# Diamondfan/CTC_pytorch

Measured on AMD Instinct MI355X. Metric: acoustic frames/sec/GPU (train) + utterances/sec beam-decode (`decode` object), TIMIT 4x320 BiLSTM, higher is better.
Workload: dtype f32 via bf16x3 split-operand MFMA (f32 accumulate); 1 GPU; cfg2: 4x320 BiLSTM + BN + Linear(62) + CTC, B=32/GPU, T=800, F=40, dropout 0.1, Adam; global_batch=32, seq_len=800, parallelism=dp1, full_length_utterances=True, sync_bn=False

## Files before the change

### ctc_pytorch_amd/_lib.py

```python
import ctypes
import glob
import os
import subprocess

import torch

_HERE = os.path.dirname(os.path.abspath(__file__))
_CSRC = os.path.join(_HERE, "csrc")
SO_PATH = os.environ.get("CTCN_LIBCTCN") or os.path.join(_HERE, "libctcn.so")
_lib = None

c_void_p, c_int, c_float, c_double, c_size_t, c_u64 = (ctypes.c_void_p, ctypes.c_int, ctypes.c_float,
                                                      ctypes.c_double, ctypes.c_size_t, ctypes.c_uint64)

P, I, F, D, Z, U = c_void_p, c_int, c_float, c_double, c_size_t, c_u64
_SIGS = {
    "ctcn_version": (I, []),
    "ctcn_last_error": (ctypes.c_char_p, []),
    "ctcn_device_cus": (I, []),
    "ctcn_device_xcds": (I, []),
    "ctcn_set_option": (I, [ctypes.c_char_p, I]),
    "ctcn_get_option": (I, [ctypes.c_char_p]),
    "ctcn_option_name": (ctypes.c_char_p, [I]),
    "ctcn_set_status_buffer": (I, [P]),
    "ctcn_gemm": (I, [I, I, I, I, I, P, I, P, I, P, I, F, I, P, Z, P]),
    "ctcn_transpose01": (I, [P, P, I, I, I, P]),
    "ctcn_copy_strided4": (I, [P, P, I, I, I, I, Z, Z, Z, Z, P]),
    "ctcn_relu_fwd": (I, [P, P, Z, P]),
    "ctcn_relu_bwd": (I, [P, P, P, Z, P]),
    "ctcn_maxpool2d_fwd": (I, [P, P, P, Z, I, I, I, I, P]),
    "ctcn_maxpool2d_bwd": (I, [P, P, P, Z, I, I, I, I, P]),
    "ctcn_rnn_scratch_bytes": (Z, [I, I, I, I]),
    "ctcn_rnn_fwd": (I, [I, I, I, I, I, I, P, P, P, P, P, P, P, P, I, P, Z, P]),
    "ctcn_rnn_fwd_dropout": (I, [I, I, I, I, I, I, P, P, P, P, P, P, P, P, P, F, U, U, I, P, Z, P]),
    "ctcn_rnn_bwd": (I, [I, I, I, I, I, I, P, P, P, P, P, P, P, P, P, P, P, P, P, P, F, I, P, P, Z, P]),
    "ctcn_rnn_bwd_dropout": (I, [I, I, I, I, I, I, P, P, P, P, P, P, P, P, P, P, P, P, P, P, F, I, P, P, Z, P, F, U, U, P]),
    "ctcn_rnn_bwd_weights": (I, [I, I, I, I, I, I, P, P, P, P, P, P, P, P, F, I, ctypes.c_uint, P, Z, P]),
    "ctcn_bn_ws_bytes": (Z, [I, I, I]),
    "ctcn_bn_fwd_train": (I, [P, P, P, P, P, P, P, P, I, I, I, F, F, I, P, Z, P, P]),
    "ctcn_bn_fwd_eval": (I, [P, P, P, P, P, P, I, I, I, F, I, P]),
    "ctcn_bn_fwd_sums": (I, [P, P, I, I, I, P, Z, P]),
    "ctcn_bn_fwd_finish": (I, [P, P, P, P, P, P, P, P, P, D, I, I, I, F, F, I, P, P]),
    "ctcn_bn_bwd_sums": (I, [P, P, P, P, P, P, I, I, I, I, P, Z, P]),
    "ctcn_bn_bwd_finish": (I, [P, P, P, P, P, P, P, P, P, P, P, D, I, I, I, I, F, P, Z, P]),
    "ctcn_bn_bwd": (I, [P, P, P, P, P, P, P, P, P, I, I, I, I, F, P, Z, P]),
    "ctcn_bn_fwd_train_dropout": (I, [P, P, P, P, P, P, P, P, I, I, I, F, F, I, P, Z, P, P, F, U, U]),
    "ctcn_bn_bwd_dropout": (I, [P, P, P, P, P, P, P, P, P, I, I, I, I, F, P, Z, P, F, U, U]),
    "ctcn_dropout": (I, [P, P, Z, F, U, U, P]),
    "ctcn_bn_masked_ws_bytes": (Z, [I, I, I]),
    "ctcn_mask_frames": (I, [P, P, P, I, I, I, I, I, P]),
    "ctcn_bn_fwd_train_masked": (I, [P, P, P, P, P, P, P, P, P, I, I, I, I, I, F, F, I, P, Z, P, P]),
    "ctcn_bn_fwd_eval_masked": (I, [P, P, P, P, P, P, P, I, I, I, I, I, F, I, P]),
    "ctcn_bn_bwd_masked": (I, [P, P, P, P, P, P, P, P, P, P, I, I, I, I, I, I, F, P, Z, P]),
    "ctcn_conv2d_ws_bytes": (Z, [I] * 11),
    "ctcn_conv2d_fwd": (I, [P, P, P, P] + [I] * 11 + [P]),
    "ctcn_conv2d_bwd": (I, [P, P, P, P, P, P] + [I] * 11 + [F, P, Z, P]),
    "ctcn_bctf_to_tbcf": (I, [P, P, I, I, I, I, P]),
    "ctcn_tbcf_to_bctf": (I, [P, P, I, I, I, I, P]),
# ... 8 lines not shown
    "ctcn_ctc_grad": (I, [P, P, P, P, P, P, P, P, P, I, I, I, I, P]),
    "ctcn_sum_f32": (I, [P, P, I, P]),
    "ctcn_ctc_fwd_ex": (I, [P, P, P, P, P, P, P, I, I, I, I, I, P]),
    "ctcn_ctc_grad_ex": (I, [P, P, P, P, P, P, P, P, I, I, I, I, P, I, I, I, I, P]),
    "ctcn_ctc_reduce": (I, [P, P, P, I, I, I, P]),
    "ctcn_ctc_pack_targets": (I, [P, ctypes.c_int64, P, P, I, I, P]),
    "ctcn_ctc_align_ws_bytes": (Z, [I, I, I]),
    "ctcn_ctc_align": (I, [P, P, P, P, P, P, P, P, P, P, I, I, I, I, I, P, Z, P]),
    "ctcn_adam_step": (I, [P, P, P, P, Z, F, F, F, F, F, I, P]),
    "ctcn_grad_norm_ws_bytes": (Z, [Z, I]),
    "ctcn_grad_norm": (I, [P, Z, I, P, I, P, P, P, I, P, Z, P]),
    "ctcn_clip_control": (I, [P, F, F, F, F, I, P]),
    "ctcn_adam_step_ex": (I, [P, P, P, P, Z, F, F, F, F, P, P]),
    "ctcn_scale_by_device_scalar": (I, [P, Z, P, P]),
    "ctcn_greedy_collapse": (I, [P, Z, Z, P, P, P, I, I, I, P]),
    "ctcn_path_tokens": (I, [P, Z, Z, P, P, P, P, P, P, P, P, P, P, I, I, I, I, P]),
    "ctcn_edit_distance": (I, [P, P, P, P, P, I, I, I, I, P]),
    "ctcn_edit_ops_ws_bytes": (Z, [I, I, I]),
    "ctcn_edit_ops": (I, [P, P, P, P, P, I, P, P, P, P, I, I, I, I, P, Z, P]),
    "ctcn_step_stats": (I, [P, P, P, I, P, P, P]),
    "ctcn_fbank_frames": (I, [ctypes.c_longlong, I, I, I]),
    "ctcn_fbank_plan_bytes": (Z, [P]),
    "ctcn_fbank_plan": (I, [P, P, Z]),
    "ctcn_fbank": (I, [P, I, P, P, P, P, P, P, P, I, I, I, F, U, U, P]),
    "ctcn_cmvn_accumulate_ws_bytes": (Z, [I, I, I]),
    "ctcn_cmvn_accumulate": (I, [P, P, P, I, I, I, P, Z, P]),
    "ctcn_comm_unique_id": (I, [P]),
    "ctcn_comm_init": (I, [P, I, I, ctypes.POINTER(ctypes.c_void_p)]),
    "ctcn_comm_allreduce_sum_f32": (I, [P, P, Z, P]),
    "ctcn_comm_destroy": (I, [P]),
    "ctcn_diag_squat": (I, [I, I, I, ctypes.c_uint, P]),
    "ctcn_diag_pipeline_chunks": (I, [I, I, I, I, I, I, I, I, ctypes.c_uint]),
    "ctcn_diag_gemm_plan": (I, [I] * 13 + [Z, ctypes.c_uint, I, I, I, I, P]),
    "ctcn_diag_gemm_on_xcds": (I, [I, I, I, I, I, P, I, P, I, P, I, F, I, P, Z, P, ctypes.c_uint]),
    "ctcn_rnn_last_kernel": (ctypes.c_char_p, [I]),
    "ctcn_levenshtein": (ctypes.c_longlong, [P, ctypes.c_longlong, P, ctypes.c_longlong]),
    "ctcn_levenshtein_ops": (ctypes.c_longlong, [P, ctypes.c_longlong, P, ctypes.c_longlong, P, P]),
    "ctcn_join_tokens": (ctypes.c_longlong, [P, ctypes.c_longlong, P, I, P, P, P, I, I, P, ctypes.c_longlong, P]),
    "ctcn_beam_ws_bytes": (Z, [I, I, I, I]),
    "ctcn_beam_decode": (I, [P, I, P, P, D, I, I, P, P, P, P, I, I, I, P, Z, P]),
    "ctcn_beam_decode_nbest": (I, [P, I, P, P, D, I, I, I, P, P, P, P, P, I, I, I, P, Z, P]),
}


class RnnCall(ctypes.Structure):
    _fields_ = [("drop_p", ctypes.c_float), ("drop_seed", ctypes.c_uint64), ("drop_offset", ctypes.c_uint64), ("y_drop", ctypes.c_void_p),
                ("dy_tmp", ctypes.c_void_p), ("side_stream", ctypes.c_void_p), ("side_event", ctypes.c_void_p), ("side_ws", ctypes.c_void_p),
                ("side_ws_bytes", ctypes.c_size_t), ("xcd_allow", ctypes.c_uint), ("prelaunch_event", ctypes.c_void_p), ("status", ctypes.c_void_p),
                ("launched", ctypes.POINTER(ctypes.c_char_p))]


class FbankOpts(ctypes.Structure):
    _fields_ = [(k, ctypes.c_float) for k in ("samp_freq", "frame_shift_ms", "frame_length_ms", "preemph_coeff", "blackman_coeff", "low_freq",
                                              "high_freq", "energy_floor")] + \
               [(k, ctypes.c_int32) for k in ("window_type", "num_mel_bins", "remove_dc_offset", "round_to_power_of_two", "snip_edges",
                                              "use_energy", "raw_energy", "htk_compat", "use_log_fbank", "use_power")]


def sources():
    return sorted(glob.glob(os.path.join(_CSRC, "*.hip")))


def build(force=False, verbose=False):
    from concurrent.futures import ThreadPoolExecutor
    srcs = sources()
    hdrs = glob.glob(os.path.join(_CSRC, "*.h")) + [os.path.join(os.path.dirname(_HERE), "include", "ctcn.h")]
# ... 101 lines not shown
```

### ctc_pytorch_amd/csrc/core.hip

```cpp
#include "common.h"

static thread_local char g_err[512] = "";

void ctcn_set_error(const char *fmt, ...) {
  va_list ap;
  va_start(ap, fmt);
  vsnprintf(g_err, sizeof(g_err), fmt, ap);
  va_end(ap);
}

extern "C" int ctcn_version(void) { return 100; }
extern "C" const char *ctcn_last_error(void) { return g_err; }
extern "C" int ctcn_device_cus(void) {
  int dev = 0, n = 0;
  if (hipGetDevice(&dev) != hipSuccess) return -1;
  if (hipDeviceGetAttribute(&n, hipDeviceAttributeMultiprocessorCount, dev) != hipSuccess) return -1;
  return n;
}

static int g_opt_rnn_persistent = 1;
static int g_opt_handoff = 1;
static int g_opt_poll_depth = 2;
static int g_opt_recurrence_only = 0;
static int g_opt_bwd_scatter = 1;
static int g_opt_handoff_tags = 1;
static int g_opt_side_split_wgs = 8;
static int g_opt_gemm_big_tiles = 0;
static int g_opt_gemm_tile256 = 1;
static int g_opt_gemm_dbg = 0;
static int g_opt_gemm_a_inline = 1;
static int g_opt_conv_mfma = 1;
static int g_opt_rnn_mixed_slices = 0;
static int g_opt_rnn_fwd_tagged = 1;
static int g_opt_rnn_fused_dropout = 1;
static int g_opt_gemm_tn = 1;
static int g_opt_tag_poll_delay = 8;
static int g_opt_edit_wave = 1;
static int g_opt_bwd_item_gather = 1;
static int g_opt_bwd_poll_delay = -1;
static int g_opt_fwd_rsv_lds = 2;
static int g_opt_fwd_pipe_any_chunking = 0;
static int g_opt_fwd_pipe_min_input = 0;
static int g_opt_conv_dbg = 0;
static int g_opt_rnn_rsv_nt = 0;
static int g_opt_gemm_bf16_single = 0;
static int g_opt_xcd_interleave = 1;
static int g_opt_bn_rows4 = 1;
static int g_opt_tn_splits_force = 0;
static int g_opt_tn_splits_xcd = 1;
static int g_opt_beam_generic_threads = 0;
static int g_opt_beam_bitonic = 1;
static int g_opt_beam_cand_global = 0;
static int g_opt_beam_occ2 = 0;
static int g_opt_beam_fast = 1;
static int g_opt_rnn_slow_items = 0;
static int g_opt_rnn_slow_exchange = 0;
static int g_opt_xcd_interleave_force = 0;
static int *g_status_dev = nullptr;

struct OptionRow { const char *name; int *var; int (*norm)(int); };
static const OptionRow k_options[] = {
  {"rnn_persistent", &g_opt_rnn_persistent, [](int value) -> int { return value; }},
  {"handoff", &g_opt_handoff, [](int value) -> int { return value; }},
  {"poll_depth", &g_opt_poll_depth, [](int value) -> int { return value; }},
  {"rnn_recurrence_only", &g_opt_recurrence_only, [](int value) -> int { return value ? 1 : 0; }},
  {"bwd_scatter", &g_opt_bwd_scatter, [](int value) -> int { return value ? 1 : 0; }},
  {"handoff_tags", &g_opt_handoff_tags, [](int value) -> int { return value ? 1 : 0; }},
  {"side_split_wgs", &g_opt_side_split_wgs, [](int value) -> int { return value < 1 ? 1 : (value > 16 ? 16 : value); }},
  {"gemm_big_tiles", &g_opt_gemm_big_tiles, [](int value) -> int { return value ? 1 : 0; }},
  {"beam_fast", &g_opt_beam_fast, [](int value) -> int { return value ? 1 : 0; }},
  {"conv_dbg", &g_opt_conv_dbg, [](int value) -> int { return value & 7; }},
  {"rnn_rsv_nt", &g_opt_rnn_rsv_nt, [](int value) -> int { return value ? 1 : 0; }},
  {"tn_splits_xcd", &g_opt_tn_splits_xcd, [](int value) -> int { return value ? 1 : 0; }},
  {"xcd_interleave", &g_opt_xcd_interleave, [](int value) -> int { return value < 0 ? 0 : (value > 5 ? 5 : value); }},
  {"bn_rows4", &g_opt_bn_rows4, [](int value) -> int { return value ? 1 : 0; }},
  {"tn_splits_force", &g_opt_tn_splits_force, [](int value) -> int { return value < 0 ? 0 : value; }},
  {"gemm_bf16_single", &g_opt_gemm_bf16_single, [](int value) -> int { return value ? 1 : 0; }},
  {"beam_generic_threads", &g_opt_beam_generic_threads, [](int value) -> int { return (value == 256 || value == 512 || value == 1024) ? value : 0; }},
  {"beam_cand_global", &g_opt_beam_cand_global, [](int value) -> int { return value ? 1 : 0; }},
  {"beam_bitonic", &g_opt_beam_bitonic, [](int value) -> int { return value ? 1 : 0; }},
  {"beam_occ2", &g_opt_beam_occ2, [](int value) -> int { return value < 0 ? 0 : (value > 2 ? 2 : value); }},
  {"fwd_pipe_min_input", &g_opt_fwd_pipe_min_input, [](int value) -> int { return value < 0 ? 0 : value; }},
  {"fwd_pipe_any_chunking", &g_opt_fwd_pipe_any_chunking, [](int value) -> int { return value ? 1 : 0; }},
  {"fwd_rsv_lds", &g_opt_fwd_rsv_lds, [](int value) -> int { return value < 0 ? 0 : (value > 2 ? 2 : value); }},
  {"bwd_item_gather", &g_opt_bwd_item_gather, [](int value) -> int { return value < 0 ? 0 : (value > 2 ? 2 : value); }},
  {"bwd_poll_delay", &g_opt_bwd_poll_delay, [](int value) -> int { return value < 0 ? -1 : (value > 256 ? 256 : value); }},
  {"conv_mfma", &g_opt_conv_mfma, [](int value) -> int { return value ? 1 : 0; }},
  {"edit_wave", &g_opt_edit_wave, [](int value) -> int { return value ? 1 : 0; }},
  {"gemm_tn", &g_opt_gemm_tn, [](int value) -> int { return value != 0; }},
  {"rnn_fused_dropout", &g_opt_rnn_fused_dropout, [](int value) -> int { return value != 0; }},
  {"tag_poll_delay", &g_opt_tag_poll_delay, [](int value) -> int { return value < 0 ? 0 : (value > 64 ? 64 : value); }},
  {"rnn_fwd_tagged", &g_opt_rnn_fwd_tagged, [](int value) -> int { return value ? 1 : 0; }},
  {"rnn_mixed_slices", &g_opt_rnn_mixed_slices, [](int value) -> int { return value ? 1 : 0; }},
  {"gemm_a_inline", &g_opt_gemm_a_inline, [](int value) -> int { return value ? 1 : 0; }},
  {"gemm_dbg", &g_opt_gemm_dbg, [](int value) -> int { return value; }},
  {"gemm_tile256", &g_opt_gemm_tile256, [](int value) -> int { return value ? 1 : 0; }},
  {"xcd_interleave_force", &g_opt_xcd_interleave_force, [](int value) -> int { return value ? 1 : 0; }},
  {"rnn_slow_exchange", &g_opt_rnn_slow_exchange, [](int value) -> int { return value < 0 ? 0 : (value > 4096 ? 4096 : value); }},
  {"rnn_slow_items", &g_opt_rnn_slow_items, [](int value) -> int { return value < 0 ? 0 : (value > 4096 ? 4096 : value); }},
};
static const int k_noptions = (int)(sizeof(k_options) / sizeof(k_options[0]));
static const OptionRow *find_option(const char *name) {
  if (name)
    for (int i = 0; i < k_noptions; ++i)
      if (!strcmp(name, k_options[i].name)) return &k_options[i];
  return nullptr;
}
extern "C" int ctcn_set_option(const char *name, int value) {
  if (const OptionRow *o = find_option(name)) { *o->var = o->norm(value); return CTCN_OK; }
  ctcn_set_error("ctcn_set_option: unknown option %s", name ? name : "(null)");
// ... 18 lines not shown
```

### ctc_pytorch_amd/csrc/gemm.hip

```cpp
#include <algorithm>
#include <type_traits>

#include "common.h"

namespace {

constexpr int BM = 128, BN = 128, BK = 16, PAD = 4;

__device__ __forceinline__ int xcd_band_tile(int bid, int nt) {
  const int xcd = bid & 7, q = nt >> 3, r = nt & 7;
  return (xcd < r ? xcd * (q + 1) : r * (q + 1) + (xcd - r) * q) + (bid >> 3);
}
__device__ __forceinline__ void g2r_kc(const float *__restrict__ src, int ld, int r0, int R, int k0, int Kend,
                                       bool vec, int tid, float (&reg)[8]) {
#pragma unroll
  for (int j = 0; j < 2; ++j) {
    const int idx = tid + 256 * j;
    const int r = idx >> 2, kq = (idx & 3) * 4;
    const int gr = r0 + r, gk = k0 + kq;
    const float *p = src + (size_t)gr * ld + gk;
    if (vec && gr < R && gk + 3 < Kend) {
      const float4 v = *reinterpret_cast<const float4 *>(p);
      reg[4 * j + 0] = v.x; reg[4 * j + 1] = v.y; reg[4 * j + 2] = v.z; reg[4 * j + 3] = v.w;
    } else {
// ... 953 lines not shown
    }
#ifdef CTCN_GEMM_STATS
    PPB_VM(2);
#else
    __builtin_amdgcn_sched_barrier(0);
    if constexpr (HAS2) asm volatile("s_waitcnt vmcnt(2) lgkmcnt(0)\n\ts_barrier" ::: "memory");
    else asm volatile("s_waitcnt vmcnt(0) lgkmcnt(0)\n\ts_barrier" ::: "memory");
    __builtin_amdgcn_sched_barrier(0);
#endif
    multiply(second, has1, has2, s);
    PPB(3);
  };
  int s = 0;
  for (; s + 2 < nst; ++s) stage(s, yes, yes);
#ifdef CTCN_GEMM_STATS
  if (lane == 0 && (wave & 3) == 0 && (blockIdx.x == 0 || blockIdx.x == 1000) && g_gemm_stats) {
    long long *o = g_gemm_stats + ((blockIdx.x ? 2 : 0) + (wave >> 2)) * 16;
    for (int i = 0; i < 4; ++i) { o[i] = gs_work[i]; o[4 + i] = gs_wait[i]; }
    o[8] = clock64() - gs_t0; o[9] = nst - 2; o[10] = 0;
  }
#endif
  if (s + 1 < nst) { stage(s, yes, no); ++s; }
  stage(s, no, no);
  if (wm == 0) pp_barrier();
#pragma unroll
  for (int i = 0; i < 4; ++i)
#pragma unroll
    for (int j = 0; j < WNT; ++j) {
      const int col = n0 + wn * 32 * WNT + j * 32 + (lane & 31);
#pragma unroll
      for (int e = 0; e < 16; ++e) {
        const int row = m0 + wm * 128 + i * 32 + (e & 3) + 8 * (e >> 2) + 4 * (lane >> 5);
        if (row < M && col < N) {
          float v = acc[i][j][e];
          float *p = C + (size_t)row * ldc + col;
          if (beta != 0.0f) v += beta * *p;
          *p = v;
        }
      }
    }
}


typedef short s16x4_t __attribute__((ext_vector_type(4)));
typedef short s16x8_t __attribute__((ext_vector_type(8)));

template <int WNT, int NP = 3>
__global__ __launch_bounds__(512) void gemm_tn_f32_pp_kernel(int M, int N, int K, const float *__restrict__ A, int lda, const float *__restrict__ B,
                                                             int ldb, float *__restrict__ C, int ldc, float beta, int kchunk, int splits,
                                                             float *__restrict__ part, int tiles_m, int tiles_n, unsigned xcd_mask,
                                                             unsigned *__restrict__ queue) {
  constexpr int TBM = 256, TBN = 128 * WNT;
  constexpr int A_BYTES = TBM * 64, B_BYTES = TBN * 64;
  constexpr int STAGE = 2 * A_BYTES + 2 * B_BYTES;
  constexpr int NB = 2 * WNT;
  constexpr int NMM = 4 * WNT;
  extern __shared__ __attribute__((aligned(16))) unsigned char qsm[];
  __shared__ int s_item;
  {
    unsigned xcc;
    asm volatile("s_getreg_b32 %0, hwreg(HW_REG_XCC_ID)" : "=s"(xcc));
    if (!((xcd_mask >> (xcc & 15u)) & 1u)) return;
  }
  const int tid = threadIdx.x, lane = tid & 63, wave = __builtin_amdgcn_readfirstlane(tid >> 6);
  const int wm = wave >> 2, wn = wave & 3;
  const int nt = tiles_m * tiles_n;
// ... 560 lines not shown
  return CTCN_OK;
}

int ctcn_gemm_on_xcds(int transA, int transB, int M, int N, int K, const float *A, int lda, const float *B, int ldb, float *C,
                      int ldc, float beta, int precision, void *ws, size_t ws_bytes, void *stream, unsigned xcd_allow, GemmPlanes *planes) {
  return gemm_core(transA, transB, M, N, K, A, lda, B, ldb, C, ldc, beta, precision, ws, ws_bytes, stream, xcd_allow, planes, 0);
}
extern "C" int ctcn_diag_gemm_on_xcds(int transA, int transB, int M, int N, int K, const float *A, int lda, const float *B, int ldb, float *C, int ldc,
                                      float beta, int precision, void *ws, size_t ws_bytes, void *stream, unsigned xcd_allow) {
  return gemm_core(transA, transB, M, N, K, A, lda, B, ldb, C, ldc, beta, precision, ws, ws_bytes, stream, xcd_allow, nullptr, 0);
}

int ctcn_gemm_shift_b(int M, int N, int K, const float *A, int lda, const float *B, int ldb, float *C, int ldc, float beta, int precision,
                      void *ws, size_t ws_bytes, void *stream, unsigned xcd_allow, int shift, GemmPlanes *planes) {
  const int as = shift < 0 ? -shift : shift;
  CTCN_REQUIRE(as < K, "ctcn_gemm_shift_b: |shift| %d >= K %d", as, K);
  const GemmEnv e = {(int)((uintptr_t)A & 15), (int)((uintptr_t)B & 15), ws != nullptr, ws_bytes, xcd_allow, false, false, ctcn_device_cus(), 0, gemm_options()};
  const bool plane = uses_planes(plan_gemm({1, 0, M, N, K, lda, ldb, ldc, precision, shift}, e).path) &&
                     plan_gemm({1, 0, M, N, K - as, lda, ldb, ldc, precision, 0}, e).path != GP_TN;
  if (!plane) {
    if (planes) planes->same_a = false;
    const float *A2 = shift > 0 ? A + (size_t)as * lda : A, *B2 = shift < 0 ? B + (size_t)as * ldb : B;
    return gemm_core(1, 0, M, N, K - as, A2, lda, B2, ldb, C, ldc, beta, precision, ws, ws_bytes, stream, xcd_allow, planes, 0);
  }
  return gemm_core(1, 0, M, N, K, A, lda, B, ldb, C, ldc, beta, precision, ws, ws_bytes, stream, xcd_allow, planes, shift);
}

extern "C" int ctcn_gemm(int transA, int transB, int M, int N, int K, const float *A, int lda, const float *B,
                         int ldb, float *C, int ldc, float beta, int precision, void *ws, size_t ws_bytes,
                         void *stream) {
  return gemm_core(transA, transB, M, N, K, A, lda, B, ldb, C, ldc, beta, precision, ws, ws_bytes, stream, 0u, nullptr, 0);
}

__global__ void transpose01_pair_kernel(const float *__restrict__ in0, const float *__restrict__ in1, float *__restrict__ out0, float *__restrict__ out1,
                                        int A, int B, int C) {
  const float *in = blockIdx.y ? in1 : in0;
  float *out = blockIdx.y ? out1 : out0;
  const size_t total = (size_t)A * B * C;
  for (size_t i = blockIdx.x * (size_t)blockDim.x + threadIdx.x; i < total; i += (size_t)gridDim.x * blockDim.x) {
    const int c = i % C;
    const size_t ab = i / C;
    const int a = ab % A;
    const int b = ab / A;
    out[i] = in[((size_t)a * B + b) * C + c];
  }
}
__global__ __launch_bounds__(256) void transpose2d_pair_kernel(const float *__restrict__ in0, const float *__restrict__ in1, float *__restrict__ out0,
                                                               float *__restrict__ out1, int A, int B) {
  __shared__ float tile[32][33];
  const float *in = blockIdx.z ? in1 : in0;
  float *out = blockIdx.z ? out1 : out0;
  const int tx = threadIdx.x & 31, ty = threadIdx.x >> 5;
  const int b0 = blockIdx.x * 32, a0 = blockIdx.y * 32;
#pragma unroll
  for (int k = 0; k < 4; ++k) {
    const int a = a0 + ty + 8 * k, b = b0 + tx;
    if (a < A && b < B) tile[ty + 8 * k][tx] = in[(size_t)a * B + b];
  }
  __syncthreads();
#pragma unroll
  for (int k = 0; k < 4; ++k) {
    const int b = b0 + ty + 8 * k, a = a0 + tx;
    if (a < A && b < B) out[(size_t)b * A + a] = tile[tx][ty + 8 * k];
  }
}
int ctcn_transpose01_pair(const float *in0, const float *in1, float *out0, float *out1, int A, int B, int C, void *stream) {
// ... 22 lines not shown
```

### ctc_pytorch_amd/csrc/rnn.hip

```cpp
#include <algorithm>
#include <stdlib.h>

#include <atomic>

#include "common.h"
#include <type_traits>

namespace {

__device__ __forceinline__ float act_sigmoid(float x) { return __builtin_amdgcn_rcpf(1.0f + __builtin_amdgcn_exp2f(-1.4426950408889634f * x)); }
__device__ __forceinline__ float act_tanh(float x) {
  const float e = __builtin_amdgcn_exp2f(-2.8853900817779268f * fabsf(x));
  return copysignf((1.0f - e) * __builtin_amdgcn_rcpf(1.0f + e), x);
}

typedef __bf16 bf16x8_t __attribute__((ext_vector_type(8)));
union Bf16Pack { u32x4 u; bf16x8_t v; };
__device__ __forceinline__ void split8(const f32x4 &a, const f32x4 &b, bf16x8_t &hi, bf16x8_t &lo) {
  unsigned h[8], l[8];
#pragma unroll
  for (int e = 0; e < 8; ++e) {
    const float x = e < 4 ? a[e] : b[e - 4];
    h[e] = f2bf(x);
    l[e] = f2bf(x - __uint_as_float(h[e] << 16));
// ... 2371 lines not shown
  bool drop_pending = c.y_drop != nullptr;
  const int rc = rnn_fwd_impl(cell, T, B, I, H, dirs, x, w_ih0, w_hh0, w_ih1, w_hh1, y, gates, aux, precision, ws, ws_bytes, stream, c, drop_pending);
  if (rc) return rc;
  return drop_pending ? ctcn_dropout(y, c.y_drop, (size_t)T * B * dirs * H, c.drop_p, c.drop_seed, c.drop_offset, stream) : CTCN_OK;
}
extern "C" int ctcn_rnn_fwd(int cell, int T, int B, int I, int H, int dirs, const float *x, const float *w_ih0,
                            const float *w_hh0, const float *w_ih1, const float *w_hh1, float *y, float *gates,
                            float *aux, int precision, void *ws, size_t ws_bytes, void *stream) {
  return ctcn_rnn_fwd_ex(cell, T, B, I, H, dirs, x, w_ih0, w_hh0, w_ih1, w_hh1, y, gates, aux, precision, ws, ws_bytes, stream, nullptr);
}
extern "C" int ctcn_rnn_fwd_dropout(int cell, int T, int B, int I, int H, int dirs, const float *x, const float *w_ih0, const float *w_hh0,
                                    const float *w_ih1, const float *w_hh1, float *y, float *gates, float *aux, float *y_drop, float p, uint64_t seed,
                                    uint64_t offset, int precision, void *ws, size_t ws_bytes, void *stream) {
  CTCN_REQUIRE(y_drop && p >= 0.0f && p < 1.0f, "ctcn_rnn_fwd_dropout: y_drop NULL or p=%f outside [0,1)", (double)p);
  ctcn_rnn_call c = {};
  c.y_drop = y_drop; c.drop_p = p; c.drop_seed = seed; c.drop_offset = offset;
  return ctcn_rnn_fwd_ex(cell, T, B, I, H, dirs, x, w_ih0, w_hh0, w_ih1, w_hh1, y, gates, aux, precision, ws, ws_bytes, stream, &c);
}

static int rnn_bwd_gemms(int cell, int T, int B, int I, int H, int dirs, const float *x, const float *w_ih0, const float *w_ih1,
                         const float *y, const float *gates, const float *aux, float *dx, float *dw_ih0, float *dw_hh0, float *dw_ih1,
                         float *dw_hh1, float beta_w, int precision, bool weights, unsigned xcd_allow, void *ws, size_t ws_bytes,
                         void *stream) {
  const int G = gates_of(cell), GH = G * H, TB = T * B;
  const float *w_ih[2] = {w_ih0, w_ih1};
  float *dw_ih[2] = {dw_ih0, dw_ih1};
  float *dw_hh[2] = {dw_hh0, dw_hh1};
  GemmPlanes pl;
  bool dx_done = false;
  if (dx && dirs == 2) {
    StackedWih s;
    if (int rc = stack_w_ih(w_ih0, w_ih1, GH, I, ws, ws_bytes, (hipStream_t)stream, s)) return rc;
    if (s.w) {
      if (int rc = ctcn_gemm_on_xcds(0, 0, TB, I, 2 * GH, gates, 2 * GH, s.w, I, dx, I, 0.0f, precision, s.ws, s.ws_bytes, stream, xcd_allow)) return rc;
      dx_done = true;
    }
  }
  for (int d = 0; d < dirs; ++d) {
    const float *da = gates + (size_t)d * GH;
    const int ldg = dirs * GH;
    int rc;
    if (dx && !dx_done) {
      rc = ctcn_gemm_on_xcds(0, 0, TB, I, GH, da, ldg, w_ih[d], I, dx, I, d == 0 ? 0.0f : 1.0f, precision, ws, ws_bytes, stream, xcd_allow);
      if (rc) return rc;
    }
    if (!weights || !dw_ih[d]) continue;
    rc = ctcn_gemm_on_xcds(1, 0, GH, I, TB, da, ldg, x, I, dw_ih[d], I, beta_w, precision, ws, ws_bytes, stream, xcd_allow, &pl);
    if (rc) return rc;
    const int Kh = (T - 1) * B;
    if (Kh <= 0) {
      if (beta_w == 0.0f) CTCN_HIP(hipMemsetAsync(dw_hh[d], 0, (size_t)GH * H * sizeof(float), (hipStream_t)stream));
      continue;
    }
    const size_t offA = d == 0 ? (size_t)B : 0, offY = d == 0 ? 0 : (size_t)B;
    const float *yh = y + (size_t)d * H + offY * dirs * H;
    if (cell == CTCN_CELL_GRU) {
      rc = ctcn_gemm_on_xcds(1, 0, 2 * H, H, Kh, da + offA * ldg, ldg, yh, dirs * H, dw_hh[d], H, beta_w, precision, ws, ws_bytes, stream, xcd_allow);
      if (rc) return rc;
      const float *dn = aux + (size_t)d * H + offA * dirs * H;
      rc = ctcn_gemm_on_xcds(1, 0, H, H, Kh, dn, dirs * H, yh, dirs * H, dw_hh[d] + (size_t)2 * H * H, H, beta_w, precision, ws, ws_bytes, stream, xcd_allow);
      if (rc) return rc;
    } else {
      pl.same_a = true;
      rc = ctcn_gemm_shift_b(GH, H, TB, da, ldg, y + (size_t)d * H, dirs * H, dw_hh[d], H, beta_w, precision, ws, ws_bytes, stream, xcd_allow,
                             d == 0 ? B : -B, &pl);
      if (rc) return rc;
    }
// ... 199 lines not shown
```

### ctc_pytorch_amd/ops.py

```python
import collections
import ctypes
import os
import numpy as np

import torch

from . import _lib

CELL = {"lstm": 0, "gru": 1, "tanh": 2}
GATES = {0: 4, 1: 3, 2: 1}

def _precision_from_env():
    v = os.environ.get("CTCN_PRECISION", "1").strip()
    if v not in ("0", "1"):
        raise ValueError("CTCN_PRECISION must be 0 (exact f32 MFMA) or 1 (bf16x3 split-operand MFMA), got %r" % v)
    return int(v)


DEFAULT_PRECISION = _precision_from_env()
_precision = [DEFAULT_PRECISION]


def set_precision(p):
    if int(p) not in (0, 1):
# ... 307 lines not shown
    return _Contiguous.apply(x)


class _BctfToTbcf(torch.autograd.Function):

    @staticmethod
    def forward(ctx, x):
        _need_gpu(x)
        x = _f32c(x)
        B, C, T, Fq = x.shape
        ctx.shape = (B, C, T, Fq)
        out = torch.empty((T, B, C * Fq), dtype=torch.float32, device=x.device)
        _lib.check(_lib.lib().ctcn_bctf_to_tbcf(_ptr(x), _ptr(out), B, C, T, Fq, _lib.stream_ptr()), "bctf_to_tbcf")
        return out

    @staticmethod
    def backward(ctx, g):
        B, C, T, Fq = ctx.shape
        g = _f32c(g)
        out = torch.empty((B, C, T, Fq), dtype=torch.float32, device=g.device)
        _lib.check(_lib.lib().ctcn_tbcf_to_bctf(_ptr(g), _ptr(out), B, C, T, Fq, _lib.stream_ptr()), "tbcf_to_bctf")
        return out


def bctf_to_tbcf(x):
    return _BctfToTbcf.apply(x)


def gemm(transA, transB, M, N, K, A, lda, Bm, ldb, C, ldc, beta=0.0, xcd_allow=0):
    _need_gpu(A, Bm, C)
    w, wp, wn = _ws(C)
    args = (int(transA), int(transB), M, N, K, _ptr(A), lda, _ptr(Bm), ldb, _ptr(C), ldc, float(beta), get_precision(), wp, wn, _lib.stream_ptr())
    _lib.check(_lib.lib().ctcn_diag_gemm_on_xcds(*args, int(xcd_allow)) if xcd_allow else _lib.lib().ctcn_gemm(*args), "gemm")
    return C


class _Linear(torch.autograd.Function):

    @staticmethod
    def forward(ctx, x, w):
        _need_gpu(x, w)
        ctx.gw_view = _gview(w)
        x, w = _f32c(x), _f32c(w)
        M, K = x.shape
        N = w.shape[0]
        y = torch.empty((M, N), dtype=torch.float32, device=x.device)
        gemm(0, 1, M, N, K, x, K, w, K, y, N)
        ctx.save_for_backward(x, w)
        return y

    @staticmethod
    def backward(ctx, gy):
        x, w = ctx.saved_tensors
        gy = _f32c(gy)
        M, K = x.shape
        N = w.shape[0]
        gx = gw = None
        if ctx.needs_input_grad[0]:
            gx = torch.empty((M, K), dtype=torch.float32, device=x.device)
            gemm(0, 0, M, K, N, gy, N, w, K, gx, K)
        if ctx.needs_input_grad[1]:
            if ctx.gw_view is not None:
                gemm(1, 0, N, K, M, gy, N, x, K, ctx.gw_view, K, beta=1.0)
            else:
                gw = torch.empty((N, K), dtype=torch.float32, device=x.device)
                gemm(1, 0, N, K, M, gy, N, x, K, gw, K)
# ... 1253 lines not shown
```

### include/ctcn.h

```cpp
#ifndef CTCN_H
#define CTCN_H
#include <stddef.h>
#include <stdint.h>
#ifdef __cplusplus
extern "C" {
#endif

#define CTCN_OK 0
#define CTCN_EINVAL (-1)
#define CTCN_EHIP (-2)
#define CTCN_EUNSUPPORTED (-3)
#define CTCN_EWORKSPACE (-4)

#define CTCN_REDUCTION_NONE 0
#define CTCN_REDUCTION_MEAN 1
#define CTCN_REDUCTION_SUM 2

#define CTCN_CELL_LSTM 0
#define CTCN_CELL_GRU 1
#define CTCN_CELL_TANH 2

int ctcn_version(void);
const char *ctcn_last_error(void);
int ctcn_device_cus(void);
int ctcn_device_xcds(void);
int ctcn_set_option(const char *name, int value);
int ctcn_get_option(const char *name);
const char *ctcn_option_name(int index);
int ctcn_set_status_buffer(int *dev_word);

int ctcn_gemm(int transA, int transB, int M, int N, int K, const float *A, int lda, const float *B, int ldb,
              float *C, int ldc, float beta, int precision, void *ws, size_t ws_bytes, void *stream);

int ctcn_transpose01(const float *in, float *out, int A, int B, int C, void *stream);
int ctcn_copy_strided4(const float *in, float *out, int d0, int d1, int d2, int d3, size_t s0, size_t s1, size_t s2,
                       size_t s3, void *stream);
int ctcn_relu_fwd(const float *x, float *y, size_t n, void *stream);
int ctcn_relu_bwd(const float *y, const float *dy, float *dx, size_t n, void *stream);
int ctcn_maxpool2d_fwd(const float *x, float *y, unsigned char *arg, size_t planes, int Hi, int Wi, int kh, int kw, void *stream);
int ctcn_maxpool2d_bwd(const float *dy, const unsigned char *arg, float *dx, size_t planes, int Hi, int Wi, int kh, int kw, void *stream);

size_t ctcn_rnn_scratch_bytes(int cell, int B, int H, int dirs);
int ctcn_rnn_fwd(int cell, int T, int B, int I, int H, int dirs, const float *x, const float *w_ih0,
                 const float *w_hh0, const float *w_ih1, const float *w_hh1, float *y, float *gates, float *aux,
                 int precision, void *ws, size_t ws_bytes, void *stream);
int ctcn_rnn_fwd_dropout(int cell, int T, int B, int I, int H, int dirs, const float *x, const float *w_ih0, const float *w_hh0,
                         const float *w_ih1, const float *w_hh1, float *y, float *gates, float *aux, float *y_drop, float p, uint64_t seed,
                         uint64_t offset, int precision, void *ws, size_t ws_bytes, void *stream);
int ctcn_rnn_bwd(int cell, int T, int B, int I, int H, int dirs, const float *x, const float *w_ih0,
                 const float *w_hh0, const float *w_ih1, const float *w_hh1, const float *y, float *gates,
                 float *aux, const float *dy, float *dx, float *dw_ih0, float *dw_hh0, float *dw_ih1,
                 float *dw_hh1, float beta_w, int precision, void *scratch, void *ws, size_t ws_bytes,
                 void *stream);
int ctcn_rnn_bwd_dropout(int cell, int T, int B, int I, int H, int dirs, const float *x, const float *w_ih0, const float *w_hh0,
                         const float *w_ih1, const float *w_hh1, const float *y, float *gates, float *aux, const float *dy, float *dx,
                         float *dw_ih0, float *dw_hh0, float *dw_ih1, float *dw_hh1, float beta_w, int precision, void *scratch, void *ws,
                         size_t ws_bytes, void *stream, float p, uint64_t seed, uint64_t offset, float *dy_tmp);
typedef struct ctcn_rnn_call {
  float drop_p;
  uint64_t drop_seed, drop_offset;
  float *y_drop;
  float *dy_tmp;
  void *side_stream, *side_event, *side_ws;
  size_t side_ws_bytes;
  unsigned xcd_allow;
// ... 134 lines not shown
                  size_t ws_bytes, void *stream);
int ctcn_step_stats(const float *loss, const int32_t *dist, const int64_t *tgt_len, int B, const int32_t *status, double *out4, void *stream);

typedef struct ctcn_fbank_opts {
  float samp_freq, frame_shift_ms, frame_length_ms, preemph_coeff, blackman_coeff, low_freq, high_freq, energy_floor;
  int32_t window_type, num_mel_bins, remove_dc_offset, round_to_power_of_two, snip_edges, use_energy, raw_energy, htk_compat, use_log_fbank,
      use_power;
} ctcn_fbank_opts;
int ctcn_fbank_frames(long long num_samples, int frame_length, int frame_shift, int snip_edges);
size_t ctcn_fbank_plan_bytes(const ctcn_fbank_opts *opts);
int ctcn_fbank_plan(const ctcn_fbank_opts *opts, void *plan, size_t plan_bytes);
int ctcn_fbank(const void *wave, int wave_is_int16, const int32_t *lens, const ctcn_fbank_opts *opts, const void *plan, const float *mean,
               const float *scale, float *feats, int32_t *frames, int B, int Nmax, int Tmax, float dither, uint64_t seed, uint64_t utt_offset,
               void *stream);
size_t ctcn_cmvn_accumulate_ws_bytes(int B, int Tmax, int F);
int ctcn_cmvn_accumulate(const float *feats, const int32_t *frames, double *stats, int B, int Tmax, int F, void *ws, size_t ws_bytes,
                         void *stream);

size_t ctcn_beam_ws_bytes(int T, int B, int V, int W);
int ctcn_beam_decode(const float *x, int input_is_prob, const int32_t *lens, const double *lm, double alpha,
                     int W, int blank, int32_t *out_ids, int32_t *out_len, double *out_score, int32_t *status,
                     int T, int B, int V, void *ws, size_t ws_bytes, void *stream);
int ctcn_beam_decode_nbest(const float *x, int input_is_prob, const int32_t *lens, const double *lm, double alpha,
                           int W, int blank, int nbest, int32_t *out_ids, int32_t *out_len, double *out_score,
                           int32_t *out_count, int32_t *status, int T, int B, int V, void *ws, size_t ws_bytes, void *stream);

int ctcn_diag_squat(int wgs_per_xcd, int threads, int lds_bytes, unsigned usec, void *stream);
int ctcn_diag_pipeline_chunks(int cell, int T, int B, int I, int H, int dirs, int xcds, int cus, unsigned xcd_allow);
#define CTCN_GEMM_PLAN_INTS 12
int ctcn_diag_gemm_plan(int transA, int transB, int M, int N, int K, int lda, int ldb, int ldc, int precision, int b_shift, int a_mod16,
                        int b_mod16, int has_ws, size_t ws_bytes, unsigned xcd_allow, int same_a, int same_b, int cus, int xcds, int *out);
int ctcn_diag_gemm_on_xcds(int transA, int transB, int M, int N, int K, const float *A, int lda, const float *B, int ldb, float *C, int ldc,
                           float beta, int precision, void *ws, size_t ws_bytes, void *stream, unsigned xcd_allow);
const char *ctcn_rnn_last_kernel(int which);

long long ctcn_join_tokens(const int32_t *ids, long long row_stride, const int32_t *lens, int B, const char *words, const int32_t *word_off,
                           const int32_t *word_len, int V, int sep, char *out, long long out_cap, long long *out_off);
long long ctcn_levenshtein(const int32_t *a, long long na, const int32_t *b, long long nb);
long long ctcn_levenshtein_ops(const int32_t *hyp, long long nh, const int32_t *ref, long long nr, long long *counts4, int32_t *ali);

#ifdef __cplusplus
}
#endif
#endif
```

Before: 1.968 million frames/s.

## Add wide 256x320-tile bf16x3 GEMM for RNN input-gradient dx path

Adds a dedicated ping-pong GEMM kernel with 256x320 tiles for the RNN backward dx product (N=320 hidden input width). The kernel converts fp32 A to bf16 hi/lo on the fly and pre-splits B into planes. A cost model picks this kernel over the generic 128-wide tiling when fewer tile waves across CUs win. The aim is to cut redundant A reads and the extra tile waves, at the cost of larger LDS use and more registers per workgroup. It is used only when no XCD restriction is set.

```diff
diff --git a/ctc_pytorch_amd/_lib.py b/ctc_pytorch_amd/_lib.py
--- a/ctc_pytorch_amd/_lib.py
+++ b/ctc_pytorch_amd/_lib.py
@@ -24,6 +24,7 @@
     "ctcn_option_name": (ctypes.c_char_p, [I]),
     "ctcn_set_status_buffer": (I, [P]),
     "ctcn_gemm": (I, [I, I, I, I, I, P, I, P, I, P, I, F, I, P, Z, P]),
+    "ctcn_gemm_dx": (I, [I, I, I, P, I, P, I, P, I, F, I, P, Z, P]),
     "ctcn_transpose01": (I, [P, P, I, I, I, P]),
     "ctcn_copy_strided4": (I, [P, P, I, I, I, I, Z, Z, Z, Z, P]),
     "ctcn_relu_fwd": (I, [P, P, Z, P]),
@@ -98,6 +99,7 @@
     "ctcn_diag_squat": (I, [I, I, I, ctypes.c_uint, P]),
     "ctcn_diag_pipeline_chunks": (I, [I, I, I, I, I, I, I, I, ctypes.c_uint]),
     "ctcn_diag_gemm_plan": (I, [I] * 13 + [Z, ctypes.c_uint, I, I, I, I, P]),
+    "ctcn_diag_dx_plan": (I, [I, I, I, I, I, I, I, Z, I, P]),
     "ctcn_diag_gemm_on_xcds": (I, [I, I, I, I, I, P, I, P, I, P, I, F, I, P, Z, P, ctypes.c_uint]),
     "ctcn_rnn_last_kernel": (ctypes.c_char_p, [I]),
     "ctcn_levenshtein": (ctypes.c_longlong, [P, ctypes.c_longlong, P, ctypes.c_longlong]),
diff --git a/ctc_pytorch_amd/csrc/core.hip b/ctc_pytorch_amd/csrc/core.hip
--- a/ctc_pytorch_amd/csrc/core.hip
+++ b/ctc_pytorch_amd/csrc/core.hip
@@ -44,6 +44,7 @@
 static int g_opt_conv_dbg = 0;
 static int g_opt_rnn_rsv_nt = 0;
 static int g_opt_gemm_bf16_single = 0;
+static int g_opt_gemm_dx_wide = 1;
 static int g_opt_xcd_interleave = 1;
 static int g_opt_bn_rows4 = 1;
 static int g_opt_tn_splits_force = 0;
@@ -76,6 +77,7 @@
   {"bn_rows4", &g_opt_bn_rows4, [](int value) -> int { return value ? 1 : 0; }},
   {"tn_splits_force", &g_opt_tn_splits_force, [](int value) -> int { return value < 0 ? 0 : value; }},
   {"gemm_bf16_single", &g_opt_gemm_bf16_single, [](int value) -> int { return value ? 1 : 0; }},
+  {"gemm_dx_wide", &g_opt_gemm_dx_wide, [](int value) -> int { return value < 0 ? 0 : (value > 2 ? 2 : value); }},
   {"beam_generic_threads", &g_opt_beam_generic_threads, [](int value) -> int { return (value == 256 || value == 512 || value == 1024) ? value : 0; }},
   {"beam_cand_global", &g_opt_beam_cand_global, [](int value) -> int { return value ? 1 : 0; }},
   {"beam_bitonic", &g_opt_beam_bitonic, [](int value) -> int { return value ? 1 : 0; }},
diff --git a/ctc_pytorch_amd/csrc/gemm.hip b/ctc_pytorch_amd/csrc/gemm.hip
--- a/ctc_pytorch_amd/csrc/gemm.hip
+++ b/ctc_pytorch_amd/csrc/gemm.hip
@@ -1009,6 +1009,218 @@
       for (int e = 0; e < 16; ++e) {
         const int row = m0 + wm * 128 + i * 32 + (e & 3) + 8 * (e >> 2) + 4 * (lane >> 5);
         if (row < M && col < N) {
+          float v = acc[i][j][e];
+          float *p = C + (size_t)row * ldc + col;
+          if (beta != 0.0f) v += beta * *p;
+          *p = v;
+        }
+      }
+    }
+}
+
+__global__ __launch_bounds__(512) void gemm_af32_n320pp_kernel(int M, int N, int K, int Kp, const float *__restrict__ A, int lda,
+                                                               const unsigned short *__restrict__ Bh, const unsigned short *__restrict__ Bl,
+                                                               float *__restrict__ C, int ldc, float beta, int tiles_m, int tiles_n) {
+  constexpr int TBM = 256, TBN = 320, WI = 2, WJ = 5;
+  constexpr int A_BYTES = TBM * 64, B_BYTES = TBN * 64;
+  constexpr int STAGE = 2 * A_BYTES + 2 * B_BYTES;
+  constexpr int NBP = 2 * TBN / 16 / 8;
+  extern __shared__ __attribute__((aligned(16))) unsigned char qsm[];
+  const int tid = threadIdx.x, lane = tid & 63, wave = __builtin_amdgcn_readfirstlane(tid >> 6);
+  const int wm = wave >> 1, wn = wave & 1;
+  const int bid = xcd_band_tile(blockIdx.x, tiles_m * tiles_n);
+  const int tm = bid / tiles_n, tn = bid - tm * tiles_n;
+  const int m0 = tm * TBM, n0 = tn * TBN;
+
+  f32x16 acc[WI][WJ];
+#pragma unroll
+  for (int i = 0; i < WI; ++i)
+#pragma unroll
+    for (int j = 0; j < WJ; ++j)
+#pragma unroll
+      for (int e = 0; e < 16; ++e) acc[i][j][e] = 0.0f;
+
+  const unsigned short *const bplane = (wave & 1) ? Bl : Bh;
+  const int bdst = 2 * A_BYTES + (wave & 1) * B_BYTES + (wave >> 1) * 1024;
+  const unsigned offB = ((unsigned)(n0 + (wave >> 1) * 16 + (lane >> 2)) * (unsigned)Kp + (unsigned)(((lane & 3) ^ ((lane >> 4) & 3)) * 8)) * 2u;
+  typedef __attribute__((address_space(3))) unsigned char *lds_u8_t;
+  auto issue_b_piece = [&](int n, int k0, int buf) {
+    const unsigned short *sbase = bplane + (size_t)n * 64 * Kp + k0;
+    const unsigned dst = (unsigned)(uintptr_t)(lds_u8_t)(qsm + buf * STAGE + bdst + n * 4096);
+    asm volatile("s_mov_b32 m0, %0\n\ts_nop 0\n\tglobal_load_lds_dwordx4 %1, %2" : : "s"(dst), "v"(offB), "s"(sbase) : "memory");
+  };
+  const int arow0 = tid >> 2, ach = tid & 3;
+  u32x4 aw[4];
+  const float *atile = A + (size_t)m0 * lda;
+  const unsigned arel[2] = {(unsigned)min(arow0, M - 1 - m0) * (unsigned)lda, (unsigned)min(128 + arow0, M - 1 - m0) * (unsigned)lda};
+  auto load_a_piece = [&](int q, int k0) {
+    const int c = 8 * ach + 4 * (q & 1);
+    const bool whole = k0 + 32 <= K;
+    const float *sbase = atile + (whole ? k0 : 0);
+    const unsigned voff = (arel[q >> 1] + (unsigned)(whole ? c : min(k0 + c, K - 4))) * 4u;
+    asm volatile("global_load_dwordx4 %0, %1, %2" : "+v"(aw[q]) : "v"(voff), "s"(sbase) : "memory");
+  };
+  auto split_pair = [](float a, float b, unsigned &hw, unsigned &lw) {
+    typedef __bf16 bf16x2_t __attribute__((ext_vector_type(2)));
+    typedef float f32x2_t __attribute__((ext_vector_type(2)));
+    hw = __builtin_bit_cast(unsigned, __builtin_convertvector((f32x2_t){a, b}, bf16x2_t));
+    const f32x2_t r = {a - __uint_as_float(hw << 16), b - __uint_as_float(hw & 0xffff0000u)};
+    lw = __builtin_bit_cast(unsigned, __builtin_convertvector(r, bf16x2_t));
+  };
+  auto convert_half = [&](int r, int h, int k0) {
+    u32x4 w = aw[2 * r + h];
+    if (k0 + 32 > K && k0 + 8 * ach + 4 * h >= K) w = (u32x4){0u, 0u, 0u, 0u};
+    unsigned h0, l0, h1, l1;
+    split_pair(__uint_as_float(w[0]), __uint_as_float(w[1]), h0, l0);
+    split_pair(__uint_as_float(w[2]), __uint_as_float(w[3]), h1, l1);
+    aw[2 * r + h] = (u32x4){h0, h1, l0, l1};
+  };
+  auto store_a_row = [&](int r, int buf) {
+    unsigned char *sb = qsm + buf * STAGE + qswz(arow0 + 128 * r, ach);
+    typedef unsigned u32x2 __attribute__((ext_vector_type(2)));
+#pragma unroll
+    for (int h = 0; h < 2; ++h) {
+      *reinterpret_cast<u32x2 *>(sb + 8 * h) = (u32x2){aw[2 * r + h][0], aw[2 * r + h][1]};
+      *reinterpret_cast<u32x2 *>(sb + A_BYTES + 8 * h) = (u32x2){aw[2 * r + h][2], aw[2 * r + h][3]};
+    }
+  };
+  const int nst = Kp / 32;
+  const int ml = lane & 31, g = lane >> 5;
+  bf16x8_t ah[WI], al[WI], bh[WJ], bl[WJ];
+  int oa[2], ob[2];
+#pragma unroll
+  for (int ks = 0; ks < 2; ++ks) {
+    oa[ks] = qswz(wm * 64 + ml, ks * 2 + g);
+    ob[ks] = 2 * A_BYTES + qswz(wn * 160 + ml, ks * 2 + g);
+  }
+  auto load_frags = [&](int stage, int ks) {
+    const unsigned char *sb = qsm + (stage & 1) * STAGE;
+#pragma unroll
+    for (int j = 0; j < WJ; ++j) {
+      bh[j] = *reinterpret_cast<const bf16x8_t *>(sb + ob[ks] + j * 2048);
+      bl[j] = *reinterpret_cast<const bf16x8_t *>(sb + B_BYTES + ob[ks] + j * 2048);
+    }
+#pragma unroll
+    for (int i = 0; i < WI; ++i) {
+      ah[i] = *reinterpret_cast<const bf16x8_t *>(sb + oa[ks] + i * 2048);
+      al[i] = *reinterpret_cast<const bf16x8_t *>(sb + A_BYTES + oa[ks] + i * 2048);
+    }
+  };
+  constexpr int NMM = WI * WJ;
+  auto multiply = [&](auto which, auto has1, auto has2, int s) {
+    constexpr int WHICH = decltype(which)::value;
+    constexpr bool HAS1 = decltype(has1)::value, HAS2 = decltype(has2)::value;
+    constexpr int CV0 = 3 * NMM - 3;
+    static_assert(NBP <= CV0, "DMA slots and split slots of a multiply phase overlap");
+#pragma unroll
+    for (int t = 0; t < 3; ++t)
+#pragma unroll
+      for (int i = 0; i < WI; ++i)
+#pragma unroll
+        for (int j = 0; j < WJ; ++j) {
+          if (t == 0) acc[i][j] = __builtin_amdgcn_mfma_f32_32x32x16_bf16(al[i], bh[j], acc[i][j], 0, 0, 0);
+          else if (t == 1) acc[i][j] = __builtin_amdgcn_mfma_f32_32x32x16_bf16(ah[i], bl[j], acc[i][j], 0, 0, 0);
+          else acc[i][j] = __builtin_amdgcn_mfma_f32_32x32x16_bf16(ah[i], bh[j], acc[i][j], 0, 0, 0);
+          const int n = t * NMM + i * WJ + j;
+          if (n < NBP || n == CV0 || n == CV0 + 1) {
+            __builtin_amdgcn_sched_barrier(0);
+            if constexpr (WHICH == 1) {
+              if (HAS1 && n < NBP) issue_b_piece(n, (s + 1) * 32, (s + 1) & 1);
+              if (HAS1 && n == CV0) {
+                static_assert(NBP == 5, "vmcnt literals");
+                if constexpr (HAS2) WAIT_A(7, 1); else WAIT_A(5, 1);
+              }
+              if (HAS1 && n >= CV0) convert_half(1, n - CV0, (s + 1) * 32);
+            } else {
+              if (HAS2 && n == CV0) WAIT_A(2, 0);
+              if (HAS2 && n >= CV0) convert_half(0, n - CV0, (s + 2) * 32);
+            }
+            __builtin_amdgcn_sched_barrier(0);
+          }
+        }
+  };
+  constexpr std::integral_constant<int, 1> first{};
+  constexpr std::integral_constant<int, 2> second{};
+  constexpr std::integral_constant<bool, true> yes{};
+  constexpr std::integral_constant<bool, false> no{};
+#pragma unroll
+  for (int q = 0; q < 4; ++q) aw[q] = (u32x4){0u, 0u, 0u, 0u};
+#pragma unroll
+  for (int q = 0; q < 4; ++q) load_a_piece(q, 0);
+#pragma unroll
+  for (int n = 0; n < NBP; ++n) issue_b_piece(n, 0, 0);
+  WAIT_A(0, 0); WAIT_A(0, 1);
+#pragma unroll
+  for (int r = 0; r < 2; ++r) {
+    convert_half(r, 0, 0); convert_half(r, 1, 0);
+    store_a_row(r, 0);
+  }
+  if (nst > 1) {
+    asm volatile("s_waitcnt lgkmcnt(0)" ::: "memory");
+#pragma unroll
+    for (int q = 0; q < 4; ++q) load_a_piece(q, 32);
+    WAIT_A(2, 0);
+    convert_half(0, 0, 32); convert_half(0, 1, 32);
+  }
+  pp_barrier_vm();
+  if (wave >= 4) pp_barrier();
+#ifdef CTCN_GEMM_STATS
+  long long gs_work[4] = {0, 0, 0, 0}, gs_wait[4] = {0, 0, 0, 0};
+  const long long gs_t0 = clock64();
+  long long gs_prev = gs_t0;
+#endif
+  auto stage = [&](int s, auto has1, auto has2) {
+    constexpr bool HAS1 = decltype(has1)::value, HAS2 = decltype(has2)::value;
+    load_frags(s, 0);
+    if constexpr (HAS1) store_a_row(0, (s + 1) & 1);
+    if constexpr (HAS2) {
+      __builtin_amdgcn_sched_barrier(0);
+      load_a_piece(0, (s + 2) * 32); load_a_piece(1, (s + 2) * 32);
+    }
+    PPB(0);
+    multiply(first, has1, has2, s);
+    PPB(1);
+    load_frags(s, 1);
+    if constexpr (HAS1) store_a_row(1, (s + 1) & 1);
+    if constexpr (HAS2) {
+      __builtin_amdgcn_sched_barrier(0);
+      load_a_piece(2, (s + 2) * 32); load_a_piece(3, (s + 2) * 32);
+    }
+#ifdef CTCN_GEMM_STATS
+    PPB_VM(2);
+#else
+    __builtin_amdgcn_sched_barrier(0);
+    if constexpr (HAS2) asm volatile("s_waitcnt vmcnt(2) lgkmcnt(0)\n\ts_barrier" ::: "memory");
+    else asm volatile("s_waitcnt vmcnt(0) lgkmcnt(0)\n\ts_barrier" ::: "memory");
+    __builtin_amdgcn_sched_barrier(0);
+#endif
+    multiply(second, has1, has2, s);
+    PPB(3);
+  };
+  int s = 0;
+  for (; s + 2 < nst; ++s) stage(s, yes, yes);
+#ifdef CTCN_GEMM_STATS
+  if (lane == 0 && (wave & 3) == 0 && (blockIdx.x == 0 || blockIdx.x == 1000) && g_gemm_stats) {
+    long long *o = g_gemm_stats + ((blockIdx.x ? 2 : 0) + (wave >> 2)) * 16;
+    for (int i = 0; i < 4; ++i) { o[i] = gs_work[i]; o[4 + i] = gs_wait[i]; }
+    o[8] = clock64() - gs_t0; o[9] = nst - 2; o[10] = 0;
+  }
+#endif
+  if (s + 1 < nst) { stage(s, yes, no); ++s; }
+  stage(s, no, no);
+  if (wave < 4) pp_barrier();
+  int zero = 0;
+  asm volatile("" : "+v"(zero));
+  const int elane = (int)__builtin_amdgcn_mbcnt_hi(~0u, __builtin_amdgcn_mbcnt_lo(~0u, (unsigned)zero));
+#pragma unroll
+  for (int i = 0; i < WI; ++i)
+#pragma unroll
+    for (int j = 0; j < WJ; ++j) {
+      const int col = n0 + wn * 160 + j * 32 + (elane & 31);
+#pragma unroll
+      for (int e = 0; e < 16; ++e) {
+        const int row = m0 + wm * 64 + i * 32 + (e & 3) + 8 * (e >> 2) + 4 * (elane >> 5);
+        if (row < M) {
           float v = acc[i][j][e];
           float *p = C + (size_t)row * ldc + col;
           if (beta != 0.0f) v += beta * *p;
@@ -1635,6 +1847,48 @@
   return gemm_core(transA, transB, M, N, K, A, lda, B, ldb, C, ldc, beta, precision, ws, ws_bytes, stream, 0u, nullptr, 0);
 }
 
+constexpr double DX_WIDE_COST = 1.87;
+struct DxPlan { bool eligible, wide; int tiles_wide, tiles_128; };
+static DxPlan plan_dx(int M, int N, int K, int lda, int precision, int a_mod16, bool has_ws, size_t ws_bytes, int cus, int opt_wide, bool single) {
+  DxPlan p = {};
+  p.tiles_128 = ceil_div(M, 256) * ceil_div(N, 128);
+  p.eligible = precision == 1 && !single && N % 320 == 0 && K >= 64 && K % 4 == 0 && lda % 4 == 0 && a_mod16 == 0 && has_ws &&
+               ws_bytes >= plane_layout(0, N, K).bytes;
+  if (!p.eligible) return p;
+  p.tiles_wide = ceil_div(M, 256) * (N / 320);
+  const int c = std::max(cus, 1);
+  p.wide = opt_wide == 2 || (opt_wide == 1 && ceil_div(p.tiles_wide, c) * DX_WIDE_COST < (double)ceil_div(p.tiles_128, c));
+  return p;
+}
+extern "C" int ctcn_diag_dx_plan(int M, int N, int K, int lda, int precision, int a_mod16, int has_ws, size_t ws_bytes, int cus, int *out) {
+  CTCN_REQUIRE(out && M > 0 && N > 0 && K >= 0 && cus > 0 && a_mod16 >= 0 && a_mod16 < 16, "ctcn_diag_dx_plan: bad args");
+  const DxPlan p = plan_dx(M, N, K, lda, precision, a_mod16, has_ws != 0, ws_bytes, cus, ctcn_get_option("gemm_dx_wide"), bf16_single());
+  const int v[CTCN_DX_PLAN_INTS] = {p.eligible, p.wide, p.tiles_wide, p.tiles_128};
+  memcpy(out, v, sizeof(v));
+  return CTCN_OK;
+}
+extern "C" int ctcn_gemm_dx(int M, int N, int K, const float *A, int lda, const float *B, int ldb, float *C, int ldc, float beta, int precision, void *ws,
+                            size_t ws_bytes, void *stream) {
+  const GemmShape g = {0, 0, M, N, K, lda, ldb, ldc, precision, 0};
+  if (const int rc = check_gemm_shape(g)) return rc;
+  CTCN_REQUIRE(A && B && C, "ctcn_gemm_dx: null pointer");
+  CTCN_REQUIRE(!ws || (uintptr_t)ws % 16 == 0, "ctcn_gemm_dx: the workspace must be 16-byte aligned");
+  const DxPlan p = plan_dx(M, N, K, lda, precision, (int)((uintptr_t)A & 15), ws != nullptr, ws_bytes, ctcn_device_cus(), ctcn_get_option("gemm_dx_wide"),
+                           bf16_single());
+  if (!p.wide) return gemm_core(0, 0, M, N, K, A, lda, B, ldb, C, ldc, beta, precision, ws, ws_bytes, stream, 0u, nullptr, 0);
+  hipStream_t st = (hipStream_t)stream;
+  const PlaneLayout lay = plane_layout(0, N, K);
+  unsigned short *bh = (unsigned short *)ws, *bl = bh + lay.b_el;
+  launch_split(SP_TRANSPOSE, st, B, ldb, N, K, lay.Kp, bh, bl, 0, 0u, nullptr);
+  CTCN_LAUNCH_CHECK();
+  const size_t lds = (size_t)2 * (2 * 256 * 64 + 2 * 320 * 64);
+  CTCN_HIP(hipFuncSetAttribute(reinterpret_cast<const void *>(gemm_af32_n320pp_kernel), hipFuncAttributeMaxDynamicSharedMemorySize, (int)lds));
+  hipLaunchKernelGGL(gemm_af32_n320pp_kernel, dim3(p.tiles_wide), dim3(512), lds, st, M, N, K, lay.Kp, A, lda, (const unsigned short *)bh,
+                     (const unsigned short *)bl, C, ldc, beta, ceil_div(M, 256), N / 320);
+  CTCN_LAUNCH_CHECK();
+  return CTCN_OK;
+}
+
 __global__ void transpose01_pair_kernel(const float *__restrict__ in0, const float *__restrict__ in1, float *__restrict__ out0, float *__restrict__ out1,
                                         int A, int B, int C) {
   const float *in = blockIdx.y ? in1 : in0;
diff --git a/ctc_pytorch_amd/csrc/rnn.hip b/ctc_pytorch_amd/csrc/rnn.hip
--- a/ctc_pytorch_amd/csrc/rnn.hip
+++ b/ctc_pytorch_amd/csrc/rnn.hip
@@ -2427,7 +2427,8 @@
     StackedWih s;
     if (int rc = stack_w_ih(w_ih0, w_ih1, GH, I, ws, ws_bytes, (hipStream_t)stream, s)) return rc;
     if (s.w) {
-      if (int rc = ctcn_gemm_on_xcds(0, 0, TB, I, 2 * GH, gates, 2 * GH, s.w, I, dx, I, 0.0f, precision, s.ws, s.ws_bytes, stream, xcd_allow)) return rc;
+      if (int rc = xcd_allow ? ctcn_gemm_on_xcds(0, 0, TB, I, 2 * GH, gates, 2 * GH, s.w, I, dx, I, 0.0f, precision, s.ws, s.ws_bytes, stream, xcd_allow)
+                             : ctcn_gemm_dx(TB, I, 2 * GH, gates, 2 * GH, s.w, I, dx, I, 0.0f, precision, s.ws, s.ws_bytes, stream)) return rc;
       dx_done = true;
     }
   }
diff --git a/ctc_pytorch_amd/ops.py b/ctc_pytorch_amd/ops.py
--- a/ctc_pytorch_amd/ops.py
+++ b/ctc_pytorch_amd/ops.py
@@ -363,6 +363,14 @@
     w, wp, wn = _ws(C)
     args = (int(transA), int(transB), M, N, K, _ptr(A), lda, _ptr(Bm), ldb, _ptr(C), ldc, float(beta), get_precision(), wp, wn, _lib.stream_ptr())
     _lib.check(_lib.lib().ctcn_diag_gemm_on_xcds(*args, int(xcd_allow)) if xcd_allow else _lib.lib().ctcn_gemm(*args), "gemm")
+    return C
+
+
+def gemm_dx(M, N, K, A, lda, Bm, ldb, C, ldc, beta=0.0):
+    _need_gpu(A, Bm, C)
+    w, wp, wn = _ws(C)
+    _lib.check(_lib.lib().ctcn_gemm_dx(M, N, K, _ptr(A), lda, _ptr(Bm), ldb, _ptr(C), ldc, float(beta), get_precision(), wp, wn, _lib.stream_ptr()),
+               "gemm_dx")
     return C
 
 
diff --git a/include/ctcn.h b/include/ctcn.h
--- a/include/ctcn.h
+++ b/include/ctcn.h
@@ -31,6 +31,9 @@
 
 int ctcn_gemm(int transA, int transB, int M, int N, int K, const float *A, int lda, const float *B, int ldb,
               float *C, int ldc, float beta, int precision, void *ws, size_t ws_bytes, void *stream);
+
+int ctcn_gemm_dx(int M, int N, int K, const float *A, int lda, const float *B, int ldb, float *C, int ldc, float beta, int precision, void *ws,
+                 size_t ws_bytes, void *stream);
 
 int ctcn_transpose01(const float *in, float *out, int A, int B, int C, void *stream);
 int ctcn_copy_strided4(const float *in, float *out, int d0, int d1, int d2, int d3, size_t s0, size_t s1, size_t s2,
@@ -231,6 +234,8 @@
                         int b_mod16, int has_ws, size_t ws_bytes, unsigned xcd_allow, int same_a, int same_b, int cus, int xcds, int *out);
 int ctcn_diag_gemm_on_xcds(int transA, int transB, int M, int N, int K, const float *A, int lda, const float *B, int ldb, float *C, int ldc,
                            float beta, int precision, void *ws, size_t ws_bytes, void *stream, unsigned xcd_allow);
+#define CTCN_DX_PLAN_INTS 4
+int ctcn_diag_dx_plan(int M, int N, int K, int lda, int precision, int a_mod16, int has_ws, size_t ws_bytes, int cus, int *out);
 const char *ctcn_rnn_last_kernel(int which);
 
 long long ctcn_join_tokens(const int32_t *ids, long long row_stride, const int32_t *lens, int B, const char *words, const int32_t *word_off,
```

Result: faster. 1.992 million frames/s (median of 6 runs) (+1.2%).
